# Ushio/2dGaussianSplatting

Measured on AMD Instinct MI355X. Metric: train iters/sec (fwd+bwd+Adam) + PSNR vs ref; 4K img, 1M splats, higher is better.
Workload: dtype f32; 1 GPU; 4096x4096 synthetic RGB, 1000000 Gaussians, fp32 (BASELINE.json configs[3]); width=4096, height=4096, n_splats=1000000, parallelism=rowslab1, rebin_interval=0, exchange_requested=none, exchange=none

## Files before the change

2dgaussiansplatting_amd/csrc/s2d_device.h:

```cpp
#pragma once

#include <hip/hip_runtime.h>
#include <stdint.h>

#include "s2d_math.h"

namespace s2d {

struct alignas(16) ProjRec {
    float4 q0, q1, q2, q3;
};
static_assert(sizeof(ProjRec) == 64, "ProjRec must be 64 bytes");

struct TileRect {
    uint16_t tx0, tx1, ty0, ty1;
};

struct Geometry {
    int W, H;
    int row_begin;
    int row_end;
    int tiles_x;
    int trow0;
    int tiles_y;
    int num_tiles;
};

struct PairCounters {
    unsigned long long fwd_visited, fwd_active, bwd_visited, bwd_active, fwd_staged, bwd_staged, fwd_wave_execs,
        bwd_wave_execs;
    unsigned long long bwd_lane_hist[65];
    unsigned long long fwd_staged_hit;
    unsigned long long fwd_rows_hit;
    unsigned long long bwd_quadrant_execs;
};

struct DeviceStatus {
    int nonfinite;
    int first_nonfinite_iter;
    int rebin_needed;
    int pad;
};

struct SqerrJob {
    const double* tile_sqerr;
    int num_tiles;
    double* out;
    double* scratch;
};

#if defined(__HIPCC__)
__device__ __forceinline__ float as_f(int v) { return __int_as_float(v); }

__device__ __forceinline__ void raise_rebin(DeviceStatus* status, int stamp, int* host_stamp)
{
    __hip_atomic_store(&status->rebin_needed, stamp, __ATOMIC_RELAXED, __HIP_MEMORY_SCOPE_AGENT);
    if (host_stamp) __hip_atomic_store(host_stamp, stamp, __ATOMIC_RELAXED, __HIP_MEMORY_SCOPE_SYSTEM);
}

__device__ __forceinline__ ProjRec pack_proj(const Projected& p)
{
    ProjRec rec;
    rec.q0 = make_float4(p.pos_x, p.pos_y, p.a, p.b);
    rec.q1 = make_float4(p.d, p.col_r, p.col_g, p.col_b);
    rec.q2 = make_float4(p.opacity, as_f(p.begY), as_f(p.endY), p.cosT);
    const float sx2 = p.sx * p.sx, sy2 = p.sy * p.sy;
    rec.q3 = make_float4(p.sinT, 1.0f / (sx2 * p.sx), 1.0f / (sy2 * p.sy), (sx2 - sy2) / (sx2 * p.sy * p.sy));
    return rec;
}

__device__ __forceinline__ bool tile_rect_of(const Projected& p, const Geometry& g, float margin, TileRect* r)
{
    const int m = (int)margin;
    long long y0 = (long long)p.begY - m, y1 = (long long)p.endY + m;
    if (p.begY == (int)0x80000000u || p.endY == (int)0x80000000u) return false;
    if (y0 < g.row_begin) y0 = g.row_begin;
    if (y1 > g.row_end - 1) y1 = g.row_end - 1;
    if (y0 > y1) return false;
    float xlo = p.pos_x - p.hx - 1.0f - margin;
    float xhi = p.pos_x + p.hx + 1.0f + margin;
    if (!(xlo <= xhi)) return false;
    if (xhi < 0.0f || xlo > (float)(g.W - 1)) return false;
    xlo = fmaxf(xlo, 0.0f);
    xhi = fminf(xhi, (float)(g.W - 1));
    r->tx0 = (uint16_t)((int)xlo >> 4);
    r->tx1 = (uint16_t)((int)xhi >> 4);
    r->ty0 = (uint16_t)(((int)y0 >> 4) - g.trow0);
    r->ty1 = (uint16_t)(((int)y1 >> 4) - g.trow0);
    return true;
}

__device__ __forceinline__ bool rect_still_covers(const Projected& p, const Geometry& g, const TileRect& binned)
{
    TileRect r;
    if (!tile_rect_of(p, g, 0.0f, &r)) return true;
    return binned.tx0 <= binned.tx1 && r.tx0 >= binned.tx0 && r.tx1 <= binned.tx1 && r.ty0 >= binned.ty0 &&
           r.ty1 <= binned.ty1;
}
#endif

constexpr float kAnisoMargin = 1.0f;
constexpr int kRasterBatch = 64;
constexpr int kSortItemsPerThread = 16;
constexpr int kSortBlock = 256;
constexpr int kSortItemsPerBlock = kSortBlock * kSortItemsPerThread;
constexpr int kScanItemsPerThread = 8;
constexpr int kScanBlock = 256;
constexpr int kScanItemsPerBlock = kScanBlock * kScanItemsPerThread;

size_t scan_temp_words(int64_t n);
hipError_t exclusive_scan_u32(const uint32_t* in, uint32_t* out, int64_t n, uint32_t* temp, uint32_t* total_dev,
                              hipStream_t stream, uint32_t* total_host_mapped = nullptr);
size_t sort_temp_words(int64_t n);
hipError_t sort_pairs_u32(uint32_t* keys_a, uint32_t* vals_a, uint32_t* keys_b, uint32_t* vals_b, int64_t n,
                          int key_bits, uint32_t* temp, uint32_t** keys_out, uint32_t** vals_out, uint32_t* tile_first,
                          hipStream_t stream);
size_t tile_first_temp_words(int num_keys);
hipError_t launch_tile_offsets_from_first(const uint32_t* tile_first, int num_keys, uint32_t total, uint32_t* temp,
                                          uint32_t* tile_off, hipStream_t stream);

struct ContainmentCheck {
    TileRect* rects = nullptr;
    DeviceStatus* status = nullptr;
    int stamp = 0;
    int* host_stamp = nullptr;
};

struct ProjectArgs {
    const float* splats = nullptr;
    const uint8_t* held = nullptr;
    int n = 0;
    Geometry g{};
    float margin = 0.0f;
    int mode = 0;
    ProjRec* proj = nullptr;
    uint32_t* counts = nullptr;
    uint32_t* row_counts = nullptr;
    ContainmentCheck check{};
};
hipError_t launch_project(const ProjectArgs& a, hipStream_t stream);
hipError_t launch_emit_row_entries(const TileRect* rects, const uint32_t* row_offsets, const uint32_t* row_counts, int n,
                                   uint32_t* keys, uint32_t* vals, uint32_t capacity, hipStream_t stream);
hipError_t launch_emit_pairs(const TileRect* rects, const uint32_t* offsets, const uint32_t* counts, int n, Geometry g,
                             uint32_t* keys, uint32_t* vals, uint32_t capacity, hipStream_t stream);
hipError_t launch_tile_offsets(const uint32_t* sorted_keys, uint32_t num_pairs, int num_tiles,
                               uint32_t* tile_off, hipStream_t stream, uint32_t key_mask = 0xFFFFFFFFu);

constexpr int kTlMaxColumns = 512;
constexpr int kTlRowBits = 12;
size_t tl_workspace_words(uint64_t entries, int tiles_x, int tiles_y);
hipError_t launch_tile_lists_from_rows(const uint32_t* entries, const uint32_t* entry_keys, uint64_t num_entries, const uint32_t* row_off,
                                       Geometry g, uint32_t* chunk_base, uint32_t* workspace, uint32_t* tile_off, uint32_t* list,
                                       hipStream_t stream);

constexpr int kDetStride = 12;
struct DetGather {
    const TileRect* rects;
    const uint32_t* offsets;
    const uint32_t* counts;
    float* data;
    uint32_t* stamp;
    uint32_t* touched;
    uint32_t now;
    int n;
};
enum class RasterPass {
    Forward,
    Backward,
    Fused,
    ForwardRange,
    BackwardRange,
};
struct RasterArgs {
    const uint32_t* tile_off = nullptr;
    const uint32_t* list = nullptr;
    const ProjRec* proj = nullptr;
    void* image0 = nullptr;
    const void* image_ref = nullptr;
    const float4* upstream = nullptr;
    float* density = nullptr;
    unsigned long long* wave_masks = nullptr;
    uint32_t* exec_list = nullptr;
    uint32_t* tile_exec = nullptr;
    uint32_t* retire_hint = nullptr;
    float* grads = nullptr;
    double* tile_sqerr = nullptr;
    Geometry g{};
    const DeviceStatus* status = nullptr;
    int iteration = 0;
    int abort_stamp = 0;
    PairCounters* counters = nullptr;
    float4* state = nullptr;
    bool first = false;
    uint32_t* any_alive = nullptr;
    bool write_image = false;
    SqerrJob sq{};
    DetGather det{};
    bool half_images = false;
    bool count = false;
    bool exact_exp = false;
    bool need_opacity_grad = false;
    bool coverage = false;
};
hipError_t launch_raster(RasterPass pass, const RasterArgs& a, hipStream_t stream);
constexpr int kRefTermsStride = 9 * kTile * kTile;
struct RefOrder {
    const float* splats = nullptr;
    const TileRect* rects = nullptr;
    const uint32_t* offsets = nullptr;
    const uint32_t* counts = nullptr;
    int n = 0;
    float* terms = nullptr;
    uint32_t* stamp = nullptr;
    uint32_t capacity = 0;
    uint32_t now = 0;
    float* pixel_sqerr = nullptr;
};
hipError_t launch_reference_backward(const RasterArgs& a, const RefOrder& ro, hipStream_t stream);
hipError_t launch_reference_sqerr(const float* pixel_sqerr, size_t pixels, double* out, const DeviceStatus* status, int iteration,
                                  hipStream_t stream);
hipError_t launch_halo_masks(const float* splats, const uint8_t* held, int n, int world, const int* row_bounds, float margin,
                             uint32_t* masks, hipStream_t stream);
hipError_t launch_halo_commit(const uint32_t* masks, int n, int rank, uint8_t* held, uint32_t* ids, uint32_t* count_dev,
                              uint32_t* scan_work, uint32_t* scan_temp, hipStream_t stream);
hipError_t launch_compact_copy(float* base, int w, const uint32_t* ids, const uint32_t* count_dev, int n, float* compact, bool to_compact,
                               hipStream_t stream);
hipError_t launch_rows_gather(const float* base, int w, const int* ids, int count, int n, float* out, hipStream_t stream);
hipError_t launch_rows_scatter(float* base, int w, const int* ids, int count, int n, const float* in, hipStream_t stream);
hipError_t launch_grads_combine(float* grads, const int* rows, int n_rows, const int* src, int world, const float* recv,
                                int n, hipStream_t stream);
constexpr int kSqerrChunks = 64;
constexpr int kSqerrScratchDoubles = kSqerrChunks + 1;
constexpr int kSqerrSmallTiles = 1024;


#if defined(__HIPCC__)
__device__ __forceinline__ double block_sum_256(double v, double* s)
{
#pragma unroll
    for (int d = 32; d >= 1; d >>= 1) v += __shfl_down(v, d, 64);
    if ((threadIdx.x & 63) == 0) s[threadIdx.x >> 6] = v;
    __syncthreads();
    const double r = ((s[0] + s[1]) + s[2]) + s[3];
    __syncthreads();
    return r;
}

__device__ __forceinline__ double sqerr_sum_small(const double* tile_sqerr, int num_tiles, double* s4)
{
    double a = 0.0;
    for (int i = (int)threadIdx.x; i < num_tiles; i += 256)
        a += __hip_atomic_load(tile_sqerr + i, __ATOMIC_RELAXED, __HIP_MEMORY_SCOPE_AGENT);
    return block_sum_256(a, s4);
}

__device__ __forceinline__ void sqerr_reduce(const double* __restrict__ tile_sqerr, int num_tiles, double* __restrict__ out,
                                             double* scratch, int first_chunk, int chunk_stride)
{
    __shared__ double s[4];
    __shared__ bool last;
    if (num_tiles <= kSqerrSmallTiles) {
        if (first_chunk != 0) return;
        const double total = sqerr_sum_small(tile_sqerr, num_tiles, s);
        if (threadIdx.x == 0) *out = total;
        return;
    }
    unsigned long long* ticket = reinterpret_cast<unsigned long long*>(scratch + kSqerrChunks);
    const int chunk = (num_tiles + kSqerrChunks - 1) / kSqerrChunks;
    unsigned long long mine = 0;
    for (int b = first_chunk; b < kSqerrChunks; b += chunk_stride, mine++) {
        const int beg = b * chunk, end = min(beg + chunk, num_tiles);
        double a0 = 0, a1 = 0, a2 = 0, a3 = 0;
        for (int i = beg + (int)threadIdx.x; i < end; i += 1024) {
            a0 += tile_sqerr[i];
            if (i + 256 < end) a1 += tile_sqerr[i + 256];
            if (i + 512 < end) a2 += tile_sqerr[i + 512];
            if (i + 768 < end) a3 += tile_sqerr[i + 768];
        }
        const double part = block_sum_256((a0 + a1) + (a2 + a3), s);
        if (threadIdx.x == 0) __hip_atomic_store(scratch + b, part, __ATOMIC_RELAXED, __HIP_MEMORY_SCOPE_AGENT);
    }
    if (threadIdx.x == 0) {
        __threadfence();
        last = mine != 0 && atomicAdd(ticket, mine) + mine == (unsigned long long)kSqerrChunks;
    }
    __syncthreads();
    if (!last) return;
    __threadfence();
    const double p = threadIdx.x < kSqerrChunks
                         ? __hip_atomic_load(scratch + threadIdx.x, __ATOMIC_RELAXED, __HIP_MEMORY_SCOPE_AGENT)
                         : 0.0;
    const double total = block_sum_256(p, s);
    if (threadIdx.x == 0) {
        *out = total;
        *ticket = 0ull;
    }
}
#endif
hipError_t launch_sqerr_finalize(SqerrJob sq, const DeviceStatus* status, int iteration, hipStream_t stream);

hipError_t launch_init_splats(float* splats, float* adams, int n, int W, int H, hipStream_t stream);
struct AdamRates {
    float r[9];
};
struct AdamArgs {
    bool controls = false;
    AdamRates rates{};
    const uint8_t* frozen = nullptr;
    float* splats = nullptr;
    float* adams = nullptr;
    float* grads = nullptr;
    const uint32_t* held_ids = nullptr;
    const uint32_t* held_count = nullptr;
    int n = 0;
    Geometry g{};
    float beta1t = 1.0f, beta2t = 1.0f, lr = 0.0f;
    int mode = 0;
    int iteration = 0;
    ProjRec* proj = nullptr;
    bool proj_current = false;
    ContainmentCheck check{};
    uint8_t* dormant = nullptr;
    SqerrJob sq{};
    bool compact = false;
};
hipError_t launch_adam(const AdamArgs& a, hipStream_t stream);
hipError_t launch_adam_controls(const AdamArgs& a, hipStream_t stream);
hipError_t launch_synthetic_target(void* image_ref, bool half_images, int W, int H, int row_begin, int row_end, hipStream_t stream);
hipError_t launch_convert_f32_to_f16(const float4* src, void* dst, size_t pixels, hipStream_t stream);
hipError_t launch_convert_f16_to_f32(const void* src, float4* dst, size_t pixels, hipStream_t stream);
hipError_t launch_test_sincos(const float* x, int n, float* s, float* c, hipStream_t stream);

}
```

2dgaussiansplatting_amd/csrc/s2d_walk.h:

```cpp
#pragma once
#include <hip/hip_fp16.h>
#include <type_traits>

#include "s2d_device.h"

namespace s2d {

constexpr int B = kRasterBatch;
static_assert(B == 64, "lane l of a wave holds the mask of batch entry l");

constexpr uint32_t kNoHint = 0xFFFFFFFFu;
constexpr uint32_t kHintFollow = 16;

constexpr int kWaveW = 8;
constexpr int kWaveH = 64 / kWaveW;
constexpr int kWavesX = kTile / kWaveW;

__device__ __forceinline__ int tile_of_block(int bid, const Geometry& g) { return bid < g.num_tiles ? bid : -1; }

__device__ __forceinline__ unsigned long long readlane_u64(unsigned long long v, int src_lane)
{
    const uint32_t lo = __builtin_amdgcn_readlane((uint32_t)v, src_lane);
    const uint32_t hi = __builtin_amdgcn_readlane((uint32_t)(v >> 32), src_lane);
    return ((unsigned long long)hi << 32) | lo;
}

template <bool HALF>
__device__ __forceinline__ float4 load_pixel(const void* base, size_t i)
{
    if (HALF) {
        const uint2 v = reinterpret_cast<const uint2*>(base)[i];
        const float2 a = __half22float2(*reinterpret_cast<const __half2*>(&v.x));
        const float2 b = __half22float2(*reinterpret_cast<const __half2*>(&v.y));
        return make_float4(a.x, a.y, b.x, b.y);
    }
    return reinterpret_cast<const float4*>(base)[i];
}

template <bool HALF>
__device__ __forceinline__ void store_pixel(void* base, size_t i, float4 c)
{
    if (HALF) {
        const __half2 a = __floats2half2_rn(c.x, c.y), b = __floats2half2_rn(c.z, c.w);
        uint2 v;
        v.x = *reinterpret_cast<const uint32_t*>(&a);
        v.y = *reinterpret_cast<const uint32_t*>(&b);
        reinterpret_cast<uint2*>(base)[i] = v;
    } else {
        reinterpret_cast<float4*>(base)[i] = c;
    }
}

struct f2 {
    float x, y;
};
__device__ __forceinline__ f2 operator+(f2 a, f2 b) { return f2{a.x + b.x, a.y + b.y}; }
__device__ __forceinline__ f2 operator-(f2 a, f2 b) { return f2{a.x - b.x, a.y - b.y}; }
__device__ __forceinline__ f2 operator*(f2 a, f2 b) { return f2{a.x * b.x, a.y * b.y}; }
__device__ __forceinline__ f2 operator*(f2 a, float b) { return f2{a.x * b, a.y * b}; }
__device__ __forceinline__ f2 operator*(float a, f2 b) { return f2{a * b.x, a * b.y}; }
__device__ __forceinline__ f2 operator-(f2 a) { return f2{-a.x, -a.y}; }
__device__ __forceinline__ f2& operator+=(f2& a, f2 b) { a = a + b; return a; }
__device__ __forceinline__ f2 fma2(f2 a, f2 b, f2 c) { return f2{__builtin_fmaf(a.x, b.x, c.x), __builtin_fmaf(a.y, b.y, c.y)}; }
__device__ __forceinline__ f2 mk2(float a, float b)
{
    f2 r;
    r.x = a;
    r.y = b;
    return r;
}

__device__ __forceinline__ void count_add(unsigned long long* counter, unsigned long long v, int lane)
{
#pragma unroll
    for (int d = 32; d >= 1; d >>= 1) v += __shfl_down(v, d, 64);
    if (lane == 0) atomicAdd(counter, v);
}

__device__ __forceinline__ void pixel_of_thread(int tid, int* lx, int* ly)
{
    const int w = tid >> 6, lane = tid & 63;
    *lx = (w % kWavesX) * kWaveW + (lane % kWaveW);
    *ly = (w / kWavesX) * kWaveH + (lane / kWaveW);
}

__device__ __forceinline__ int stage_masks(uint32_t* s_mask32, int se, int sub, const float4& q0, const float4& q1,
                                            int begY, int endY, int y_tile, int x_tile, int W, int row_end)
{
    uint32_t rm[4];
#pragma unroll
    for (int k = 0; k < 4; k++) {
        const int yy = y_tile + sub * 4 + k;
        rm[k] = 0;
        if (yy < row_end) rm[k] = row_mask16(q0.x, q0.y, q0.z, q0.w, q1.x, begY, endY, yy, x_tile, W);
    }
    const int wy = sub >> 1, half = sub & 1;
#pragma unroll
    for (int wx = 0; wx < 2; wx++) {
        const int sh = 8 * wx;
        const uint32_t word = ((rm[0] >> sh) & 0xFFu) | (((rm[1] >> sh) & 0xFFu) << 8) |
                              (((rm[2] >> sh) & 0xFFu) << 16) | (((rm[3] >> sh) & 0xFFu) << 24);
        s_mask32[((wy * 2 + wx) * B + se) * 2 + half] = word;
    }
    return (rm[0] != 0u) + (rm[1] != 0u) + (rm[2] != 0u) + (rm[3] != 0u);
}

template <bool EXACT>
__device__ __forceinline__ float gauss_of(float d2, bool* nonzero)
{
    if (EXACT) {
        *nonzero = true;
        return expf_ref(-0.5f * d2);
    }
    return gauss_pow8(d2, nonzero);
}

struct TileCtx {
    int tile, tx, ty;
    int tid, lane, w;
    int x, y;
    bool inside;
    f2 pxy;
};

__device__ __forceinline__ TileCtx tile_ctx(int tile, const Geometry& g)
{
    TileCtx c;
    c.tile = tile;
    c.tx = tile % g.tiles_x;
    c.ty = tile / g.tiles_x + g.trow0;
    c.tid = threadIdx.x;
    c.lane = c.tid & 63;
    c.w = c.tid >> 6;
    int lx, ly;
    pixel_of_thread(c.tid, &lx, &ly);
    c.x = c.tx * kTile + lx;
    c.y = c.ty * kTile + ly;
    c.inside = c.x < g.W && c.y < g.row_end;
    c.pxy = mk2((float)c.x + 0.5f, (float)c.y + 0.5f);
    return c;
}

__device__ __forceinline__ size_t pixel_index(const TileCtx& c, const Geometry& g) { return (size_t)(c.y - g.row_begin) * g.W + c.x; }

struct FwdShared {
    float4 rec[B][3];
    unsigned long long mask[2][4 * B];
    uint32_t idx[2][B];
    unsigned long long touched[4];
    int4 alive;
};

__device__ __forceinline__ bool block_any_alive(int4* flags, int w, int lane, unsigned long long alive_mask)
{
    if (lane == 0) reinterpret_cast<int*>(flags)[w] = alive_mask != 0ull ? 1 : 0;
    __syncthreads();
    const int4 f = *flags;
    return ((f.x | f.y) | (f.z | f.w)) != 0;
}

__device__ __forceinline__ bool block_any_alive_exec(int4* flags, unsigned long long* touched4, int w, int lane,
                                                     unsigned long long alive_mask, unsigned long long touched,
                                                     unsigned long long* exec_mask)
{
    if (lane == 0) {
        reinterpret_cast<int*>(flags)[w] = alive_mask != 0ull ? 1 : 0;
        touched4[w] = touched;
    }
    __syncthreads();
    const int4 f = *flags;
    const unsigned long long m = (touched4[0] | touched4[1]) | (touched4[2] | touched4[3]);
    const uint32_t lo = __builtin_amdgcn_readfirstlane((uint32_t)m), hi = __builtin_amdgcn_readfirstlane((uint32_t)(m >> 32));
    *exec_mask = ((unsigned long long)hi << 32) | lo;
    return ((f.x | f.y) | (f.z | f.w)) != 0;
}

struct Blended {
    float cb, T;
    unsigned long long alive_mask;
};
template <bool EXACT>
__device__ __forceinline__ Blended blend_entry(const float4 q0, const float4 q1, const float4 q2, const f2 pxy, unsigned long long act,
                                               f2& crg, float cb, float T, unsigned long long alive_mask)
{
    const f2 v = pxy - mk2(q0.x, q0.y);
    const f2 m = mk2(q0.z, q0.w) * v.x + mk2(q1.x, q1.y) * v.y;
    const f2 vm = v * m;
    bool nonzero;
    const float G = gauss_of<EXACT>(vm.x + vm.y, &nonzero);
    const unsigned long long on = act & __ballot(nonzero);
    const float alpha = __builtin_amdgcn_inverse_ballot_w64(on) ? G * q2.y : 0.0f;
    crg += (T * mk2(q1.z, q1.w)) * alpha;
    cb += T * q2.x * alpha;
    T *= (1.0f - alpha);
    alive_mask &= __ballot(!(T < kMinThroughput));
    return Blended{cb, T, alive_mask};
}

struct BlendedCoverage {
    float cb, ca, T;
    unsigned long long alive_mask;
};
template <bool EXACT>
__device__ __forceinline__ BlendedCoverage blend_entry_coverage(const float4 q0, const float4 q1, const float4 q2, const f2 pxy,
                                                                unsigned long long act, f2& crg, float cb, float ca, float T,
                                                                unsigned long long alive_mask)
{
    const f2 v = pxy - mk2(q0.x, q0.y);
    const f2 m = mk2(q0.z, q0.w) * v.x + mk2(q1.x, q1.y) * v.y;
    const f2 vm = v * m;
    bool nonzero;
    const float G = gauss_of<EXACT>(vm.x + vm.y, &nonzero);
    const unsigned long long on = act & __ballot(nonzero);
    const float alpha = __builtin_amdgcn_inverse_ballot_w64(on) ? G * q2.y : 0.0f;
    crg += (T * mk2(q1.z, q1.w)) * alpha;
    cb += T * q2.x * alpha;
    ca += T * alpha;
    T *= (1.0f - alpha);
    alive_mask &= __ballot(!(T < kMinThroughput));
    return BlendedCoverage{cb, ca, T, alive_mask};
}

template <bool COUNT, bool EXACT, bool CHUNK = false, bool COVERAGE = false>
__device__ __forceinline__ uint32_t forward_tile(FwdShared& s, const TileCtx& c, const uint32_t* __restrict__ tile_off,
                                             const uint32_t* __restrict__ list, const ProjRec* __restrict__ proj,
                                             unsigned long long* __restrict__ wave_masks, uint32_t* __restrict__ exec_list,
                                             uint32_t* __restrict__ retire_hint, const Geometry& g,
                                             PairCounters* __restrict__ counters, f2& crg, float& cb, float* T_io = nullptr,
                                             float* ca_out = nullptr)
{
    static_assert(!(COVERAGE && (COUNT || EXACT || CHUNK)), "the coverage channel: plain lists, exp_approx, no pair counting");
    constexpr bool HINT = !COUNT && !CHUNK;
    const int tid = c.tid, lane = c.lane, w = c.w;
    const f2 pxy = c.pxy;
    float T = 1.0f;
    if (CHUNK) {
        T = *T_io;
    } else {
        crg = mk2(0.0f, 0.0f);
        cb = 0.0f;
    }
    [[maybe_unused]] float ca = 0.0f;
    unsigned long long alive_mask = __ballot(CHUNK ? c.inside && !(T < kMinThroughput) : c.inside);
    unsigned long long n_vis = 0, n_act = 0, n_staged = 0, n_exec = 0, n_rows_hit = 0, n_staged_hit = 0;

    const uint32_t beg = tile_off[c.tile], end = tile_off[c.tile + 1];
    const int se = tid >> 2, sub = tid & 3;
    uint32_t n_out = 0;
    uint32_t hint = kNoHint, last_exec = 0;
    bool retired = false;
    if constexpr (HINT) hint = retire_hint[c.tile];
    int pb = 1;
    for (uint32_t base = beg, cnt_u = 0; base < end; base += cnt_u) {
        uint32_t want = B;
        if constexpr (HINT) {
            const uint32_t pos = base - beg;
            if (hint != kNoHint) {
                if (hint <= pos) want = kHintFollow;
                else if (hint - pos <= (uint32_t)B) want = (hint - pos + 15u) & ~15u;
            }
        }
        cnt_u = min(want, end - base);
        const int cnt = (int)cnt_u;
        pb ^= 1;
        unsigned long long* const s_mask = s.mask[pb];
        if (se < cnt) {
            const uint32_t idx = list[base + se];
            const ProjRec* r = proj + idx;
            const float4 q0 = r->q0, q1 = r->q1, q2 = r->q2;
            const int rows_hit = stage_masks(reinterpret_cast<uint32_t*>(s_mask), se, sub, q0, q1, __float_as_int(q2.y),
                                             __float_as_int(q2.z), c.ty * kTile, c.tx * kTile, g.W, g.row_end);
            if (COUNT) {
                n_rows_hit += rows_hit;
                const int entry_rows = rows_hit + __shfl_xor(rows_hit, 1) + __shfl_xor(rows_hit, 2);
                n_staged_hit += (sub == 0 && entry_rows > 0) ? 1 : 0;
            }
            if (sub == 0) {
                s.rec[se][0] = q0;
                s.rec[se][1] = make_float4(q0.w, q1.x, q1.y, q1.z);
                s.rec[se][2] = make_float4(q1.w, q2.x, 0.0f, 0.0f);
                if (!COUNT) s.idx[pb][se] = idx;
            }
        }
        __syncthreads();
        if constexpr (COUNT) {
            if (se < cnt) wave_masks[(size_t)(base + se) * 4 + sub] = s_mask[sub * B + se];
            n_staged += (tid == 0) ? (unsigned long long)cnt : 0ull;
        }
        unsigned long long touched = 0ull;
        if (alive_mask != 0ull || COUNT) {
            const unsigned long long my_mask = (lane < cnt) ? s_mask[w * B + lane] : 0ull;
            unsigned long long cand = __ballot(COUNT ? my_mask != 0ull : (my_mask & alive_mask) != 0ull);
            while (cand != 0ull) {
                const int e = __builtin_ctzll(cand);
                cand &= cand - 1ull;
                const unsigned long long wm = readlane_u64(my_mask, e);
                if (COUNT) n_vis += (wm >> lane) & 1ull;
                const unsigned long long act = wm & alive_mask;
                if (act == 0ull) continue;
                if (COUNT) n_exec += (lane == 0);
                else touched |= 1ull << e;
                if constexpr (COVERAGE) {
                    const BlendedCoverage bl = blend_entry_coverage<EXACT>(s.rec[e][0], s.rec[e][1], s.rec[e][2], pxy, act, crg, cb, ca, T, alive_mask);
                    cb = bl.cb;
                    ca = bl.ca;
                    T = bl.T;
                    alive_mask = bl.alive_mask;
                } else {
                    const Blended bl = blend_entry<EXACT>(s.rec[e][0], s.rec[e][1], s.rec[e][2], pxy, act, crg, cb, T, alive_mask);
                    cb = bl.cb;
                    T = bl.T;
                    alive_mask = bl.alive_mask;
                }
                if (COUNT) n_act += (act >> lane) & 1ull;
            }
        }
        if constexpr (COUNT) {
            if (!block_any_alive(&s.alive, w, lane, alive_mask)) break;
        } else {
            unsigned long long exec_mask;
            const bool any = block_any_alive_exec(&s.alive, s.touched, w, lane, alive_mask, touched, &exec_mask);
            if ((exec_mask >> se) & 1ull) {
                const uint32_t at = beg + n_out + (uint32_t)__popcll(exec_mask & ((1ull << se) - 1ull));
                wave_masks[(size_t)at * 4 + sub] = s_mask[sub * B + se];
                if (sub == 0) exec_list[at] = s.idx[pb][se];
            }
            n_out += (uint32_t)__popcll(exec_mask);
            if (HINT && exec_mask != 0ull) last_exec = (base - beg) + 64u - (uint32_t)__builtin_clzll(exec_mask);
            if (!any) {
                retired = true;
                break;
            }
        }
    }
    if (CHUNK) *T_io = T;
    if constexpr (COVERAGE) *ca_out = ca;
    if constexpr (HINT)
        if (tid == 0) retire_hint[c.tile] = retired ? last_exec : kNoHint;
    if (COUNT) {
        count_add(&counters->fwd_visited, n_vis, lane);
        count_add(&counters->fwd_active, n_act, lane);
        if (tid == 0) atomicAdd(&counters->fwd_staged, n_staged);
        if (lane == 0) atomicAdd(&counters->fwd_wave_execs, n_exec);
        count_add(&counters->fwd_rows_hit, n_rows_hit, lane);
        count_add(&counters->fwd_staged_hit, n_staged_hit, lane);
    }
    return n_out;
}

__device__ __forceinline__ bool launch_is_void(const DeviceStatus* status, int abort_stamp, int iteration)
{
    return (abort_stamp != 0 && status->rebin_needed == abort_stamp) || status->first_nonfinite_iter < iteration;
}

static inline unsigned raster_grid(int num_tiles) { return (unsigned)(((num_tiles + 7) / 8) * 8); }

template <bool EXACT, bool COUNT, bool HALF, bool... MORE, typename F>
static hipError_t with_variant(F&& f)
{
    if constexpr (EXACT && (COUNT || HALF)) return hipErrorInvalidValue;
    else return f(std::bool_constant<EXACT>{}, std::bool_constant<COUNT>{}, std::bool_constant<HALF>{},
                  std::bool_constant<MORE>{}...), hipSuccess;
}
template <bool... DONE, typename F, typename... REST>
static hipError_t with_variant(F&& f, bool flag, REST... rest)
{
    return flag ? with_variant<DONE..., true>(f, rest...) : with_variant<DONE..., false>(f, rest...);
}
template <bool... DONE, typename F, bool FLAG, typename... REST>
static hipError_t with_variant(F&& f, std::bool_constant<FLAG>, REST... rest)
{
    return with_variant<DONE..., FLAG>(f, rest...);
}

hipError_t launch_raster_ranges(RasterPass pass, const RasterArgs& a, hipStream_t stream);
hipError_t launch_raster_gradient(const RasterArgs& a, hipStream_t stream);
hipError_t launch_det_gather(const RasterArgs& a, hipStream_t stream);
hipError_t launch_raster_coverage(RasterPass pass, const RasterArgs& a, hipStream_t stream);

}
```

Before: 630.6 iterations/s.

## Double the forward raster staging batch to 128 splats per sync round

The non-counting forward walk now stages 128 list entries per round instead of 64. Each thread loads two entries, the blend loop runs two 64-wide mask passes, and the compaction step handles two exec masks. The aim is to halve the number of block-wide __syncthreads rounds and amortize staging overhead per splat. In exchange it doubles shared memory per block, which may lower occupancy, and it adds wasted staging work when tiles saturate early within a batch.

```diff
diff --git a/2dgaussiansplatting_amd/csrc/s2d_device.h b/2dgaussiansplatting_amd/csrc/s2d_device.h
--- a/2dgaussiansplatting_amd/csrc/s2d_device.h
+++ b/2dgaussiansplatting_amd/csrc/s2d_device.h
@@ -101,6 +101,7 @@
 
 constexpr float kAnisoMargin = 1.0f;
 constexpr int kRasterBatch = 64;
+constexpr int kForwardBatch = 128;
 constexpr int kSortItemsPerThread = 16;
 constexpr int kSortBlock = 256;
 constexpr int kSortItemsPerBlock = kSortBlock * kSortItemsPerThread;
diff --git a/2dgaussiansplatting_amd/csrc/s2d_walk.h b/2dgaussiansplatting_amd/csrc/s2d_walk.h
--- a/2dgaussiansplatting_amd/csrc/s2d_walk.h
+++ b/2dgaussiansplatting_amd/csrc/s2d_walk.h
@@ -84,6 +84,7 @@
     *ly = (w / kWavesX) * kWaveH + (lane / kWaveW);
 }
 
+template <int NB = B>
 __device__ __forceinline__ int stage_masks(uint32_t* s_mask32, int se, int sub, const float4& q0, const float4& q1,
                                             int begY, int endY, int y_tile, int x_tile, int W, int row_end)
 {
@@ -100,7 +101,7 @@
         const int sh = 8 * wx;
         const uint32_t word = ((rm[0] >> sh) & 0xFFu) | (((rm[1] >> sh) & 0xFFu) << 8) |
                               (((rm[2] >> sh) & 0xFFu) << 16) | (((rm[3] >> sh) & 0xFFu) << 24);
-        s_mask32[((wy * 2 + wx) * B + se) * 2 + half] = word;
+        s_mask32[((wy * 2 + wx) * NB + se) * 2 + half] = word;
     }
     return (rm[0] != 0u) + (rm[1] != 0u) + (rm[2] != 0u) + (rm[3] != 0u);
 }
@@ -143,11 +144,13 @@
 
 __device__ __forceinline__ size_t pixel_index(const TileCtx& c, const Geometry& g) { return (size_t)(c.y - g.row_begin) * g.W + c.x; }
 
+constexpr int FB = kForwardBatch;
+static_assert(FB == 2 * B, "lane l of a wave holds the masks of batch entries l and l + 64");
 struct FwdShared {
-    float4 rec[B][3];
-    unsigned long long mask[2][4 * B];
-    uint32_t idx[2][B];
-    unsigned long long touched[4];
+    float4 rec[FB][3];
+    unsigned long long mask[2][4 * FB];
+    uint32_t idx[2][FB];
+    unsigned long long touched[4][2];
     int4 alive;
 };
 
@@ -159,19 +162,25 @@
     return ((f.x | f.y) | (f.z | f.w)) != 0;
 }
 
-__device__ __forceinline__ bool block_any_alive_exec(int4* flags, unsigned long long* touched4, int w, int lane,
-                                                     unsigned long long alive_mask, unsigned long long touched,
-                                                     unsigned long long* exec_mask)
+__device__ __forceinline__ unsigned long long uniform_u64(unsigned long long m)
+{
+    const uint32_t lo = __builtin_amdgcn_readfirstlane((uint32_t)m), hi = __builtin_amdgcn_readfirstlane((uint32_t)(m >> 32));
+    return ((unsigned long long)hi << 32) | lo;
+}
+__device__ __forceinline__ bool block_any_alive_exec(int4* flags, unsigned long long (*touched4)[2], int w, int lane,
+                                                     unsigned long long alive_mask, unsigned long long touched_lo,
+                                                     unsigned long long touched_hi, unsigned long long* exec_lo,
+                                                     unsigned long long* exec_hi)
 {
     if (lane == 0) {
         reinterpret_cast<int*>(flags)[w] = alive_mask != 0ull ? 1 : 0;
-        touched4[w] = touched;
+        touched4[w][0] = touched_lo;
+        touched4[w][1] = touched_hi;
     }
     __syncthreads();
     const int4 f = *flags;
-    const unsigned long long m = (touched4[0] | touched4[1]) | (touched4[2] | touched4[3]);
-    const uint32_t lo = __builtin_amdgcn_readfirstlane((uint32_t)m), hi = __builtin_amdgcn_readfirstlane((uint32_t)(m >> 32));
-    *exec_mask = ((unsigned long long)hi << 32) | lo;
+    *exec_lo = uniform_u64((touched4[0][0] | touched4[1][0]) | (touched4[2][0] | touched4[3][0]));
+    *exec_hi = uniform_u64((touched4[0][1] | touched4[1][1]) | (touched4[2][1] | touched4[3][1]));
     return ((f.x | f.y) | (f.z | f.w)) != 0;
 }
 
@@ -231,6 +240,8 @@
 {
     static_assert(!(COVERAGE && (COUNT || EXACT || CHUNK)), "the coverage channel: plain lists, exp_approx, no pair counting");
     constexpr bool HINT = !COUNT && !CHUNK;
+    constexpr int NB = COUNT ? B : FB;
+    constexpr int PASSES = NB / 64;
     const int tid = c.tid, lane = c.lane, w = c.w;
     const f2 pxy = c.pxy;
     float T = 1.0f;
@@ -252,81 +263,103 @@
     if constexpr (HINT) hint = retire_hint[c.tile];
     int pb = 1;
     for (uint32_t base = beg, cnt_u = 0; base < end; base += cnt_u) {
-        uint32_t want = B;
+        uint32_t want = NB;
         if constexpr (HINT) {
             const uint32_t pos = base - beg;
             if (hint != kNoHint) {
                 if (hint <= pos) want = kHintFollow;
-                else if (hint - pos <= (uint32_t)B) want = (hint - pos + 15u) & ~15u;
+                else if (hint - pos <= (uint32_t)NB) want = (hint - pos + 15u) & ~15u;
             }
         }
         cnt_u = min(want, end - base);
         const int cnt = (int)cnt_u;
         pb ^= 1;
         unsigned long long* const s_mask = s.mask[pb];
-        if (se < cnt) {
-            const uint32_t idx = list[base + se];
-            const ProjRec* r = proj + idx;
-            const float4 q0 = r->q0, q1 = r->q1, q2 = r->q2;
-            const int rows_hit = stage_masks(reinterpret_cast<uint32_t*>(s_mask), se, sub, q0, q1, __float_as_int(q2.y),
-                                             __float_as_int(q2.z), c.ty * kTile, c.tx * kTile, g.W, g.row_end);
-            if (COUNT) {
-                n_rows_hit += rows_hit;
-                const int entry_rows = rows_hit + __shfl_xor(rows_hit, 1) + __shfl_xor(rows_hit, 2);
-                n_staged_hit += (sub == 0 && entry_rows > 0) ? 1 : 0;
-            }
-            if (sub == 0) {
-                s.rec[se][0] = q0;
-                s.rec[se][1] = make_float4(q0.w, q1.x, q1.y, q1.z);
-                s.rec[se][2] = make_float4(q1.w, q2.x, 0.0f, 0.0f);
-                if (!COUNT) s.idx[pb][se] = idx;
+#pragma unroll 1
+        for (int e0 = 0; e0 < cnt; e0 += 64) {
+            int off = e0;
+            if (PASSES > 1) asm volatile("" : "+s"(off));
+            const int e = se + off;
+            if (e < cnt) {
+                const uint32_t idx = list[base + e];
+                const ProjRec* r = proj + idx;
+                const float4 q0 = r->q0, q1 = r->q1, q2 = r->q2;
+                const int rows_hit = stage_masks<NB>(reinterpret_cast<uint32_t*>(s_mask), e, sub, q0, q1, __float_as_int(q2.y),
+                                                     __float_as_int(q2.z), c.ty * kTile, c.tx * kTile, g.W, g.row_end);
+                if (COUNT) {
+                    n_rows_hit += rows_hit;
+                    const int entry_rows = rows_hit + __shfl_xor(rows_hit, 1) + __shfl_xor(rows_hit, 2);
+                    n_staged_hit += (sub == 0 && entry_rows > 0) ? 1 : 0;
+                }
+                if (sub == 0) {
+                    s.rec[e][0] = q0;
+                    s.rec[e][1] = make_float4(q0.w, q1.x, q1.y, q1.z);
+                    s.rec[e][2] = make_float4(q1.w, q2.x, 0.0f, 0.0f);
+                    if (!COUNT) s.idx[pb][e] = idx;
+                }
             }
         }
         __syncthreads();
         if constexpr (COUNT) {
-            if (se < cnt) wave_masks[(size_t)(base + se) * 4 + sub] = s_mask[sub * B + se];
+            if (se < cnt) wave_masks[(size_t)(base + se) * 4 + sub] = s_mask[sub * NB + se];
             n_staged += (tid == 0) ? (unsigned long long)cnt : 0ull;
         }
-        unsigned long long touched = 0ull;
-        if (alive_mask != 0ull || COUNT) {
-            const unsigned long long my_mask = (lane < cnt) ? s_mask[w * B + lane] : 0ull;
-            unsigned long long cand = __ballot(COUNT ? my_mask != 0ull : (my_mask & alive_mask) != 0ull);
-            while (cand != 0ull) {
-                const int e = __builtin_ctzll(cand);
-                cand &= cand - 1ull;
-                const unsigned long long wm = readlane_u64(my_mask, e);
-                if (COUNT) n_vis += (wm >> lane) & 1ull;
-                const unsigned long long act = wm & alive_mask;
-                if (act == 0ull) continue;
-                if (COUNT) n_exec += (lane == 0);
-                else touched |= 1ull << e;
-                if constexpr (COVERAGE) {
-                    const BlendedCoverage bl = blend_entry_coverage<EXACT>(s.rec[e][0], s.rec[e][1], s.rec[e][2], pxy, act, crg, cb, ca, T, alive_mask);
-                    cb = bl.cb;
-                    ca = bl.ca;
-                    T = bl.T;
-                    alive_mask = bl.alive_mask;
-                } else {
-                    const Blended bl = blend_entry<EXACT>(s.rec[e][0], s.rec[e][1], s.rec[e][2], pxy, act, crg, cb, T, alive_mask);
-                    cb = bl.cb;
-                    T = bl.T;
-                    alive_mask = bl.alive_mask;
+        unsigned long long touched[PASSES];
+#pragma unroll
+        for (int h = 0; h < PASSES; h++) {
+            touched[h] = 0ull;
+            if ((alive_mask != 0ull && 64 * h < cnt) || (COUNT && h == 0)) {
+                const unsigned long long my_mask = (lane + 64 * h < cnt) ? s_mask[w * NB + 64 * h + lane] : 0ull;
+                unsigned long long cand = __ballot(COUNT ? my_mask != 0ull : (my_mask & alive_mask) != 0ull);
+                while (cand != 0ull) {
+                    const int el = __builtin_ctzll(cand), e = 64 * h + el;
+                    cand &= cand - 1ull;
+                    const unsigned long long wm = readlane_u64(my_mask, el);
+                    if (COUNT) n_vis += (wm >> lane) & 1ull;
+                    const unsigned long long act = wm & alive_mask;
+                    if (act == 0ull) continue;
+                    if (COUNT) n_exec += (lane == 0);
+                    else touched[h] |= 1ull << el;
+                    if constexpr (COVERAGE) {
+                        const BlendedCoverage bl = blend_entry_coverage<EXACT>(s.rec[e][0], s.rec[e][1], s.rec[e][2], pxy, act, crg, cb, ca, T, alive_mask);
+                        cb = bl.cb;
+                        ca = bl.ca;
+                        T = bl.T;
+                        alive_mask = bl.alive_mask;
+                    } else {
+                        const Blended bl = blend_entry<EXACT>(s.rec[e][0], s.rec[e][1], s.rec[e][2], pxy, act, crg, cb, T, alive_mask);
+                        cb = bl.cb;
+                        T = bl.T;
+                        alive_mask = bl.alive_mask;
+                    }
+                    if (COUNT) n_act += (act >> lane) & 1ull;
                 }
-                if (COUNT) n_act += (act >> lane) & 1ull;
             }
         }
         if constexpr (COUNT) {
             if (!block_any_alive(&s.alive, w, lane, alive_mask)) break;
         } else {
-            unsigned long long exec_mask;
-            const bool any = block_any_alive_exec(&s.alive, s.touched, w, lane, alive_mask, touched, &exec_mask);
-            if ((exec_mask >> se) & 1ull) {
-                const uint32_t at = beg + n_out + (uint32_t)__popcll(exec_mask & ((1ull << se) - 1ull));
-                wave_masks[(size_t)at * 4 + sub] = s_mask[sub * B + se];
-                if (sub == 0) exec_list[at] = s.idx[pb][se];
-            }
-            n_out += (uint32_t)__popcll(exec_mask);
-            if (HINT && exec_mask != 0ull) last_exec = (base - beg) + 64u - (uint32_t)__builtin_clzll(exec_mask);
+            unsigned long long exec_lo, exec_hi;
+            const bool any = block_any_alive_exec(&s.alive, s.touched, w, lane, alive_mask, touched[0], touched[PASSES - 1], &exec_lo, &exec_hi);
+            int sc = se;
+            asm volatile("" : "+v"(sc));
+            const uint32_t n_lo = (uint32_t)__popcll(exec_lo);
+            const unsigned long long below = (1ull << sc) - 1ull;
+            if ((exec_lo >> sc) & 1ull) {
+                const uint32_t at = beg + n_out + (uint32_t)__popcll(exec_lo & below);
+                wave_masks[(size_t)at * 4 + sub] = s_mask[sub * NB + sc];
+                if (sub == 0) exec_list[at] = s.idx[pb][sc];
+            }
+            if ((exec_hi >> sc) & 1ull) {
+                const uint32_t at = beg + n_out + n_lo + (uint32_t)__popcll(exec_hi & below);
+                wave_masks[(size_t)at * 4 + sub] = s_mask[sub * NB + 64 + sc];
+                if (sub == 0) exec_list[at] = s.idx[pb][64 + sc];
+            }
+            n_out += n_lo + (uint32_t)__popcll(exec_hi);
+            if constexpr (HINT) {
+                if (exec_hi != 0ull) last_exec = (base - beg) + 128u - (uint32_t)__builtin_clzll(exec_hi);
+                else if (exec_lo != 0ull) last_exec = (base - beg) + 64u - (uint32_t)__builtin_clzll(exec_lo);
+            }
             if (!any) {
                 retired = true;
                 break;
```

Result: no change. 631.1 iterations/s (median of 2 runs) (+0.1%).
